# yuanqing-wang/stag

Hardware: AMD Instinct MI355X
Metric: aggregated edges/sec, stochastic-aggregation layer-forward, ogbn-arxiv-shaped CSR (higher is better)
Workload: dtype f32

## Files before the change

stag_amd/csrc/agg_kernel.hpp:

```cpp
#pragma once
#include "../../include/stag_hip.h"
#include "noise.hpp"

namespace stag {

struct AggArgs {
  const int32_t* indptr;
  const int32_t* indices;
  const int32_t* eid;
  const int32_t* nidx;
  int32_t n_rows;
  const float* x;
  int64_t ldx;
  int32_t D;
  uint32_t ldxb;
  uint32_t ldwb;
  uint32_t x_bytes;
  int32_t wide;
  const float* p0;
  const float* p1;
  float p0s, p1s;
  int32_t pmode;
  int32_t relu, in_norm;
  int32_t wgroup;
  PhiloxKey key;
  uint32_t pos_lo, pos_hi;
  uint32_t chunk_base;
  int32_t n_heavy;
  int32_t n_heavy_blocks;
  struct alignas(32) Walk {
    int32_t smask, sshift;
    int32_t jh_heavy;
    int32_t jh_light;
    int32_t sh;
    int32_t lbase;
    int32_t sl;
    int32_t n_total;
  } walk;
  const int32_t* xcd;
  const float* src_scale;
  const float* dst_scale;
  int32_t mean;
  float* out;
  float* outx[3];
  int32_t mc;
  uint64_t mc_stride;
  int64_t ldo;
  float* norm_scale_out;
  const float* xown;
  int64_t ldxo;
  const float* own_scale;
  float* eg0;
  float* eg1;
  float* dp_part;
  const stag_unit* units;
  const stag_unit* units_plan;
  int32_t n_units;
  const int32_t* long_rows;
  const int32_t* long_seg_ptr;
  int32_t n_long;
  int32_t n_seg;
  int32_t* seg_counters;
  float* ws;
  int32_t ws_stride;
  uint32_t ws_bytes;
};

__device__ __forceinline__ void load4(const float* p, int k0, int D, bool vec, float (&v)[4]) {
  if (vec) {
    const float4 t = *reinterpret_cast<const float4*>(p + k0);
    v[0] = t.x; v[1] = t.y; v[2] = t.z; v[3] = t.w;
  } else {
#pragma unroll
    for (int j = 0; j < 4; ++j) v[j] = (k0 + j < D) ? p[k0 + j] : 0.0f;
  }
}

__device__ __forceinline__ void store4(float* p, int k0, int D, bool vec, const float (&v)[4]) {
  if (vec) {
    *reinterpret_cast<float4*>(p + k0) = make_float4(v[0], v[1], v[2], v[3]);
  } else {
#pragma unroll
    for (int j = 0; j < 4; ++j)
      if (k0 + j < D) p[k0 + j] = v[j];
  }
}

__device__ __forceinline__ void store4_sc1(__amdgpu_buffer_rsrc_t rsrc, uint32_t off, int k0, int D,
                                           bool vec, const float (&v)[4]) {
  typedef unsigned int u32x4 __attribute__((ext_vector_type(4)));
  if (vec) {
    const u32x4 t = {__float_as_uint(v[0]), __float_as_uint(v[1]), __float_as_uint(v[2]),
                     __float_as_uint(v[3])};
    __builtin_amdgcn_raw_buffer_store_b128(t, rsrc, (int)off, 0, 16);
  } else {
#pragma unroll
    for (int j = 0; j < 4; ++j)
      if (k0 + j < D)
        __builtin_amdgcn_raw_buffer_store_b32(__float_as_uint(v[j]), rsrc, (int)(off + 4u * j), 0, 16);
  }
}

template <int NF, bool VEC>
__device__ __forceinline__ void kahan_sum_partials(const float* ws, int ws_stride, int s0, int s1,
                                                   int k0, int D, float (&sum)[4], float (&comp)[4]) {
  comp[0] = comp[1] = comp[2] = comp[3] = 0.f;
  sum[0] = sum[1] = sum[2] = sum[3] = 0.f;
#pragma unroll 1
  for (int s = s0; s < s1; s += NF) {
    float t[NF][4];
#pragma unroll
    for (int i = 0; i < NF; ++i) {
      if (s + i < s1) load4(ws + (int64_t)(s + i) * ws_stride, k0, D, VEC, t[i]);
      else t[i][0] = t[i][1] = t[i][2] = t[i][3] = 0.f;
    }
#pragma unroll
    for (int i = 0; i < NF; ++i)
#pragma unroll
      for (int q = 0; q < 4; ++q) {
        const float y = t[i][q] - comp[q];
        const float n = sum[q] + y;
        comp[q] = (n - sum[q]) - y;
        sum[q] = n;
      }
  }
}

__device__ __forceinline__ void agg_epilogue_extra(const AggArgs& a, float* out, int v, int deg, int k0,
                                                   bool vec, float (&acc)[4]);

constexpr int kCombineGroup = 16;
template <int NF, bool VEC, int LPE, int SLOTS>
__device__ __forceinline__ void two_level_sum(const float* ws, int ws_stride, int s0, int s1, int k0,
                                              int D, int sl, int slot0, float (&sum)[4]) {
  float comp[4] = {0.f, 0.f, 0.f, 0.f};
  sum[0] = sum[1] = sum[2] = sum[3] = 0.f;
#pragma unroll 1
  for (int g0 = s0; g0 < s1; g0 += kCombineGroup * SLOTS) {
    const int gs = g0 + sl * kCombineGroup;
    float gsum[4] = {0.f, 0.f, 0.f, 0.f}, gres[4] = {0.f, 0.f, 0.f, 0.f};
    if (gs < s1) {
      const int ge = min(gs + kCombineGroup, s1);
      kahan_sum_partials<NF, VEC>(ws, ws_stride, gs, ge, k0, D, gsum, gres);
    }
#pragma unroll
    for (int j = 0; j < SLOTS; ++j) {
      if (g0 + j * kCombineGroup < s1) {
#pragma unroll
// ... 377 lines not shown
      for (int o = 0; o < NX; ++o) fold_into(X.acc[o], X.comp[o], TX.acc[o]);
    }
    }
  }

  __device__ __forceinline__ void fold(const float (&t)[4]) { fold_into(acc, comp, t); }

  __device__ __forceinline__ void fold_into(float (&s)[4], float (&cmp)[4], const float (&t)[4]) const {
    if (kahan) {
#pragma unroll
      for (int q = 0; q < 4; ++q) {
        const float y = t[q] - cmp[q];
        const float sum = s[q] + y;
        cmp[q] = (sum - s[q]) - y;
        s[q] = sum;
      }
    } else {
#pragma unroll
      for (int q = 0; q < 4; ++q) s[q] += t[q];
    }
  }

  __device__ __forceinline__ void block_sums(EdgeRows<NB, PEDGE>& R, const EdgeIdx<NB>& I, int p0,
                                             float (&t)[MULT][4], float (&we)[NB][4]) {
#pragma unroll
    for (int m = 0; m < MULT; ++m) {
#pragma unroll
      for (int q = 0; q < 4; ++q) t[m][q] = 0.f;
#pragma unroll
      for (int j = m * BLK; j < (m + 1) * BLK; ++j) {
        if (p0 + j < pend) {
          edge_weight(R, I, j, we[j]);
          if (a.src_scale) {
            asm volatile("" ::: "memory");
#pragma unroll
            for (int q = 0; q < 4; ++q) R.xv[j][q] *= R.xs[j];
          }
#pragma unroll
          for (int q = 0; q < 4; ++q) t[m][q] = __builtin_fmaf(we[j][q], R.xv[j][q], t[m][q]);
        }
      }
    }
  }

  __device__ __forceinline__ void edge_weight(const EdgeRows<NB, PEDGE>& R, const EdgeIdx<NB>& I, int j,
                                              float (&w)[4]) {
    if constexpr (KIND == kNone) {
      w[0] = w[1] = w[2] = w[3] = 1.0f;
    } else if constexpr (KIND == kExplicit) {
      if (a.wgroup > 1) {
        const float* wr = a.p0 + (int64_t)I.ee[j] * (a.D / a.wgroup);
#pragma unroll
        for (int q = 0; q < 4; ++q) w[q] = (k0 + q < a.D) ? wr[(k0 + q) / a.wgroup] : 0.0f;
      } else {
        loadrow4(row_at(a.p0, I.ee[j], a.ldwb, koff, (a.wide & 2) != 0), k0, a.D, VEC, w);
      }
      if (a.relu & kFlagRelu) {
#pragma unroll
        for (int q = 0; q < 4; ++q) w[q] = fmaxf(w[q], 0.0f);
      }
    } else {
      if constexpr (PEDGE == 1) {
        const float s1 = (a.relu & kFlagLogScale) ? exp_scale(R.P.q1[j]) : R.P.q1[j];
#pragma unroll
        for (int q = 0; q < 4; ++q) { pa[q] = R.P.q0[j]; pb[q] = s1; }
        draw4<KIND>(I.nn[j], c1, key, pa, pb, a.relu, w);
        return;
      } else if constexpr (PEDGE == 2) {
        if (a.relu & kFlagLogScale) {
          float pbe[4];
#pragma unroll
          for (int q = 0; q < 4; ++q) pbe[q] = exp_scale(R.P.pb[j][q]);
          draw4<KIND>(I.nn[j], c1, key, R.P.pa[j], pbe, a.relu, w);
        } else {
          draw4<KIND>(I.nn[j], c1, key, R.P.pa[j], R.P.pb[j], a.relu, w);
        }
        return;
      }
      draw4<KIND>(I.nn[j], c1, key, pa, pb, a.relu, w);
    }
  }
};

template <int KIND, int LPE, bool VEC, int PEDGE, int SLOTS, int MULT, int NOUT = 1, bool MC = false, bool WN = false,
          bool NULLS = false>
__device__ __forceinline__ void agg_unit(const AggArgs& a, const int unit, const int c, const int sl,
                                         float (*dp_out)[4] = nullptr) {
  static_assert(LPE * SLOTS <= 64 && 64 % (LPE * SLOTS) == 0, "a unit's lanes stay inside one wave");
  static_assert(NOUT == 1 || SLOTS == 1, "the derivative outputs take the one-slot loop");
#ifndef STAG_BLK_EG
#define STAG_BLK_EG 1
#endif
#ifndef STAG_BLK_DP
#define STAG_BLK_DP 1
#endif
  constexpr int BLK = PEDGE == 3 ? STAG_BLK_EG : PEDGE == 4 ? STAG_BLK_DP : (KIND >= kNormal) ? STAG_BLK_RNG : STAG_BLK_MEM;
  constexpr int NB = BLK * MULT;

  const uint32_t chunk = blockIdx.y * LPE + c;
  const int k0 = (int)chunk * 4;
  if (k0 >= a.D) return;

  int v, b, len, slot = -1;
  if (a.units) {
    const int4 q = *reinterpret_cast<const int4*>(a.units + unit);
    v = q.x; b = q.y; len = q.z; slot = q.w;
    if constexpr (NULLS) {
      if (v < 0) return;
    }
  } else {
    v = unit;
    b = a.indptr[v];
    len = a.indptr[v + 1] - b;
  }

  if (len > STAG_PRIO_MIN_LEN) __builtin_amdgcn_s_setprio(2);
#ifdef STAG_TRACE
  uint64_t* trace = (!a.in_norm && a.norm_scale_out && blockIdx.y == 0 && c == 0 && sl == 0)
                        ? reinterpret_cast<uint64_t*>(a.norm_scale_out) + (int64_t)unit * 4 : nullptr;
  if (trace) { trace[0] = wall_clock64(); trace[1] = trace[2] = trace[3] = 0; }
#endif

  AggTeam<KIND, LPE, VEC, PEDGE, BLK, MULT, NOUT, MC, WN> T{
      a, (KIND >= kNormal) ? resolve_epoch(a.key) : a.key, k0, (uint32_t)k0 * 4u,
      (chunk + a.chunk_base) | (a.pos_hi << 20),
      b + len,
      __builtin_amdgcn_make_buffer_rsrc(const_cast<float*>(a.x), 0, (int)a.x_bytes, 0x00020000),
      (a.wide & 1) == 0 && a.x_bytes != 0,
      {a.p0s, a.p0s, a.p0s, a.p0s}, {a.p1s, a.p1s, a.p1s, a.p1s},
      {0.f, 0.f, 0.f, 0.f}, {0.f, 0.f, 0.f, 0.f}, {0.f, 0.f, 0.f, 0.f},
      len > kKahanMinLen};
  if constexpr (MC) {
#pragma unroll
    for (int o = 0; o < NOUT - 1; ++o) T.KX.k[o] = key_plus(T.key, (uint64_t)(o + 1) * a.mc_stride);
  }
  if constexpr (PEDGE == 3 || PEDGE == 4) {
    const int row = slot >= 0 ? a.long_rows[v] : v;
    const float os = a.own_scale ? a.own_scale[row] : 1.0f;
    if (PEDGE == 3 || a.xown) {
      load4(a.xown + (int64_t)row * a.ldxo, k0, a.D, VEC, T.XO.v);
    } else {
#pragma unroll
      for (int q = 0; q < 4; ++q) T.XO.v[q] = (k0 + q < a.D) ? 1.0f : 0.0f;
    }
#pragma unroll
    for (int q = 0; q < 4; ++q) T.XO.v[q] *= os;
  }
  if constexpr (KIND >= kNormal) {
    if (a.pmode == STAG_PARAM_PER_CHANNEL) {
      load4(a.p0, k0, a.D, VEC, T.pa);
      if (a.p1) load4(a.p1, k0, a.D, VEC, T.pb);
    }
  }

  const int pend = b + len;
  EdgeIdx<NB> I;
  EdgeRows<NB, PEDGE> R;
  {
    constexpr bool PREFETCH = STAG_IDX_PREFETCH && LPE <= ((KIND >= kNormal) ? STAG_PREFETCH_MAX_LPE : STAG_PREFETCH_MAX_LPE_MEM);
    if constexpr (SLOTS > 1) {
      constexpr int RB = SLOTS * NB;
      const int base = ((int)(threadIdx.x & 63) - sl * LPE) << 2;
      for (int r0 = b; r0 < pend; r0 += RB) {
        const int p0 = r0 + sl * NB;
#if STAG_LOAD_PRIO
        __builtin_amdgcn_s_setprio(3);
#endif
        T.fetch_idx(I, p0);
        T.pin_idx(I);
        T.fetch_rows(R, I, p0);
#if STAG_LOAD_PRIO
        if (len > STAG_PRIO_MIN_LEN) __builtin_amdgcn_s_setprio(2); else __builtin_amdgcn_s_setprio(0);
#endif
        float t[MULT][4], we[NB][4];
        T.block_sums(R, I, p0, t, we);
#pragma unroll
        for (int j = 0; j < SLOTS; ++j) {
#pragma unroll
          for (int m = 0; m < MULT; ++m) {
            const int pb = r0 + (j * MULT + m) * BLK;
            if (pb < pend) {
              float tj[4];
#pragma unroll
              for (int q = 0; q < 4; ++q)
                tj[q] = __int_as_float(__builtin_amdgcn_ds_bpermute(base + j * (LPE << 2), __float_as_int(t[m][q])));
              T.fold(tj);
              if (a.in_norm) {
#pragma unroll
                for (int e = 0; e < BLK; ++e) {
                  if (pb + e < pend) {
#pragma unroll
                    for (int q = 0; q < 4; ++q)
                      T.wsum[q] += __int_as_float(__builtin_amdgcn_ds_bpermute(
                          base + j * (LPE << 2), __float_as_int(we[m * BLK + e][q])));
                  }
                }
              }
            }
          }
        }
      }
    } else if constexpr (PREFETCH) {
    EdgeIdx<NB> In;
    T.fetch_idx(I, b);
    for (int p0 = b; p0 < pend; p0 += NB) {
#if STAG_LOAD_PRIO
      __builtin_amdgcn_s_setprio(3);
#endif
      T.pin_idx(I);
      T.fetch_rows(R, I, p0);
      if (p0 + NB < pend) T.fetch_idx(In, p0 + NB);
#if STAG_LOAD_PRIO
      if (len > STAG_PRIO_MIN_LEN) __builtin_amdgcn_s_setprio(2); else __builtin_amdgcn_s_setprio(0);
#endif
      T.compute(R, I, p0);
      I = In;
    }
    } else {
    for (int p0 = b; p0 < pend; p0 += NB) {
#if STAG_LOAD_PRIO
      __builtin_amdgcn_s_setprio(3);
#endif
      T.fetch_idx(I, p0);
      T.pin_idx(I);
      T.fetch_rows(R, I, p0);
#if STAG_LOAD_PRIO
      if (len > STAG_PRIO_MIN_LEN) __builtin_amdgcn_s_setprio(2); else __builtin_amdgcn_s_setprio(0);
#endif
      T.compute(R, I, p0);
    }
    }
  }

#ifdef STAG_TRACE
  if (trace) trace[1] = wall_clock64();
#endif
  if constexpr (PEDGE == 4) {
#pragma unroll
    for (int i = 0; i < 2; ++i)
#pragma unroll
      for (int q = 0; q < 4; ++q) dp_out[i][q] = T.DP.v[i][q];
// ... 153 lines not shown
    if constexpr (HS > 1) {
      if (blk < a.n_heavy_blocks) {
        const int unit = blk * TPBH + threadIdx.x / (LPE * HS);
        if (unit >= a.n_heavy) return;
        agg_unit<KIND, LPE, VEC, PEDGE, HS, STAG_HMULT>(a, unit, c, (threadIdx.x / LPE) % HS);
        return;
      }
      first = a.n_heavy;
      blk -= a.n_heavy_blocks;
    }
    const int unit = first + blk * TPB + threadIdx.x / LPE;
    if (unit >= a.n_units) return;
    agg_unit<KIND, LPE, VEC, PEDGE, 1, NOUT == 1 ? mult_of<KIND, LPE>() : 1, NOUT, MC, WN>(a, unit, c, 0);
  } else {
    const AggArgs::Walk w = a.walk;
    const int stripe = blockIdx.x & w.smask;
    int j = blockIdx.x >> w.sshift;
    int unit0, end;
    bool heavy = false;
    if (HS > 1 && j < w.jh_heavy) {
      heavy = true;
      unit0 = stripe * w.sh + j * TPBH;
      end = (stripe + 1) * w.sh;
    } else {
      if (HS > 1) j -= w.jh_heavy;
      if (j < w.jh_light) {
        unit0 = stripe * w.sh + j * TPB;
        end = (stripe + 1) * w.sh;
      } else {
        j -= w.jh_light;
        unit0 = w.lbase + stripe * w.sl + j * TPB;
        end = min(w.lbase + (stripe + 1) * w.sl, w.n_total);
      }
    }
    if constexpr (HS > 1) {
      if (heavy) {
        const int unit = unit0 + threadIdx.x / (LPE * HS);
        if (unit >= end) return;
        agg_unit<KIND, LPE, VEC, PEDGE, HS, STAG_HMULT, 1, false, false, true>(a, unit, c, (threadIdx.x / LPE) % HS);
        return;
      }
    }
    const int unit = unit0 + threadIdx.x / LPE;
    if (unit >= end) return;
#ifndef STAG_MULT_WALK_WIDE
#define STAG_MULT_WALK_WIDE 2
#endif
    constexpr int MULT_W = NOUT != 1 ? 1 : (KIND == kNone && PEDGE == 0 && LPE >= 64) ? STAG_MULT_WALK_WIDE : mult_of<KIND, LPE>();
    agg_unit<KIND, LPE, VEC, PEDGE, 1, MULT_W, NOUT, MC, WN, true>(a, unit, c, 0);
  }
}

template <int KIND, int LPE, bool VEC>
__global__ __launch_bounds__(STAG_BLOCK_THREADS, STAG_WAVES_PER_SIMD) void agg_dp_kernel(const AggArgs a) {
  constexpr int TEAMS = STAG_BLOCK_THREADS / LPE;
  __shared__ float s_dp[TEAMS][2][LPE * 4];
  const int c = threadIdx.x % LPE, tm = threadIdx.x / LPE;
  const int unit = blockIdx.x * TEAMS + tm;
  float dp[2][4] = {{0.f, 0.f, 0.f, 0.f}, {0.f, 0.f, 0.f, 0.f}};
  if (unit < a.n_units) agg_unit<KIND, LPE, VEC, 4, 1, 1>(a, unit, c, 0, dp);
#pragma unroll
  for (int i = 0; i < 2; ++i)
#pragma unroll
    for (int q = 0; q < 4; ++q) s_dp[tm][i][c * 4 + q] = dp[i][q];
  __syncthreads();
  float* part = a.dp_part + ((int64_t)blockIdx.y * gridDim.x + blockIdx.x) * (2 * LPE * 4);
  for (int i = threadIdx.x; i < 2 * LPE * 4; i += STAG_BLOCK_THREADS) {
    float sum = 0.f;
#pragma unroll
    for (int j = 0; j < TEAMS; ++j) sum += s_dp[j][i / (LPE * 4)][i % (LPE * 4)];
    part[i] = sum;
  }
}

template <int KIND>
hipError_t agg_launch(const AggArgs& a, bool vec, hipStream_t stream);

#ifndef STAG_XCD_PLANLESS
#define STAG_XCD_PLANLESS 1
#endif
#ifndef STAG_AGG_LDS_BYTES
#define STAG_AGG_LDS_BYTES 0
#endif
template <int KIND>
inline void agg_launch_small(const AggArgs& a_in, bool vec, int tiles, hipStream_t s) {
  AggArgs a = a_in;
  constexpr int LPE = 32, TPB = STAG_BLOCK_THREADS / LPE, TPBH = STAG_BLOCK_THREADS / (LPE * heavy_slots_of<KIND, LPE, true>());
  a.n_heavy_blocks = (a.n_heavy + TPBH - 1) / TPBH;
  const dim3 grid(a.n_heavy_blocks + (a.n_units - a.n_heavy + TPB - 1) / TPB, tiles), block(STAG_BLOCK_THREADS);
  if (grid.x == 0) return;
  if (vec) hipLaunchKernelGGL((agg_kernel<KIND, LPE, true, 0, 1, false, false, false, true>), grid, block, STAG_AGG_LDS_BYTES, s, a);
  else     hipLaunchKernelGGL((agg_kernel<KIND, LPE, false, 0, 1, false, false, false, true>), grid, block, STAG_AGG_LDS_BYTES, s, a);
}

template <int KIND, int LPE>
inline void agg_launch_shape(const AggArgs& a_in, bool vec, int pedge, int tiles, hipStream_t s) {
  if constexpr (LPE == 32 && heavy_slots_of<KIND, 32, true>() != heavy_slots_of<KIND, 32, false>()) {
    if (!a_in.outx[0] && !a_in.dp_part && pedge == 0 && !a_in.xcd && a_in.units && a_in.n_heavy > 0 &&
        a_in.n_units <= STAG_SMALL_UNITS) {
      agg_launch_small<KIND>(a_in, vec, tiles, s);
      return;
    }
  }
  AggArgs a = a_in;
  constexpr int TPB = STAG_BLOCK_THREADS / LPE;
  constexpr int HS = heavy_slots_of<KIND, LPE>();
  constexpr int TPBH = STAG_BLOCK_THREADS / (LPE * HS);
  const bool slotted = !(HS == 1 || a.outx[0] || pedge == 3 || a.dp_part);
  if (!slotted) a.n_heavy = 0;
  const bool plain = !a.outx[0] && !a.dp_part && pedge == 0;
  if (a.xcd && a.dp_part) { a.xcd = nullptr; a.units = a.units_plan; }
  a.n_heavy_blocks = (a.n_heavy + TPBH - 1) / TPBH;
  dim3 grid(a.n_heavy_blocks + (a.n_units - a.n_heavy + TPB - 1) / TPB, tiles);
  bool walk = false;
  AggArgs::Walk& w = a.walk;
  if (a.xcd) {
    walk = true;
    w.smask = STAG_XCD_STRIPES - 1; w.sshift = 3;
    w.jh_heavy = slotted ? (w.sh + TPBH - 1) / TPBH : 0;
    w.jh_light = slotted ? 0 : (w.sh + TPB - 1) / TPB;
    w.lbase = STAG_XCD_STRIPES * w.sh;
    w.n_total = STAG_XCD_STRIPES * (w.sh + w.sl);
    grid.x = STAG_XCD_STRIPES * (w.jh_heavy + w.jh_light + (w.sl + TPB - 1) / TPB);
  } else if (STAG_XCD_PLANLESS && !a.dp_part && !a.units && a.n_units >= STAG_XCD_STRIPES * TPB && a.n_units < (1 << 30)) {
    walk = true;
    w = AggArgs::Walk{STAG_XCD_STRIPES - 1, 3, 0, 0, 0, 0, 0, a.n_units};
    w.sl = ((a.n_units + STAG_XCD_STRIPES - 1) / STAG_XCD_STRIPES + TPB - 1) / TPB * TPB;
    grid.x = STAG_XCD_STRIPES * (w.sl / TPB);
  } else if (!plain && !a.dp_part) {
    walk = true;
    w = AggArgs::Walk{0, 0, 0, 0, a.n_heavy, a.n_heavy, a.n_units - a.n_heavy, a.n_units};
    w.jh_heavy = slotted ? a.n_heavy_blocks : 0;
    w.jh_light = slotted ? 0 : (w.sh + TPB - 1) / TPB;
    grid.x = w.jh_heavy + w.jh_light + (w.sl + TPB - 1) / TPB;
  }
  if (grid.x == 0) return;
  const dim3 block(STAG_BLOCK_THREADS);
  if constexpr (KIND >= kNormal) {
    if (a.mc && a.outx[2]) {
      if (vec) hipLaunchKernelGGL((agg_kernel<KIND, LPE, true, 0, 4, true, false, true>), grid, block, STAG_AGG_LDS_BYTES, s, a);
      else     hipLaunchKernelGGL((agg_kernel<KIND, LPE, false, 0, 4, true, false, true>), grid, block, STAG_AGG_LDS_BYTES, s, a);
      return;
    }
    if (a.mc && a.outx[0] && a.in_norm) {
      if (vec) hipLaunchKernelGGL((agg_kernel<KIND, LPE, true, 0, 2, true, true, true>), grid, block, STAG_AGG_LDS_BYTES, s, a);
      else     hipLaunchKernelGGL((agg_kernel<KIND, LPE, false, 0, 2, true, true, true>), grid, block, STAG_AGG_LDS_BYTES, s, a);
      return;
    }
    if (a.mc && a.outx[0]) {
      if (vec) hipLaunchKernelGGL((agg_kernel<KIND, LPE, true, 0, 2, true, false, true>), grid, block, STAG_AGG_LDS_BYTES, s, a);
      else     hipLaunchKernelGGL((agg_kernel<KIND, LPE, false, 0, 2, true, false, true>), grid, block, STAG_AGG_LDS_BYTES, s, a);
      return;
    }
  }
  if constexpr (KIND == kNormal || KIND == kUniform) {
    if (a.outx[0]) {
      if (vec) hipLaunchKernelGGL((agg_kernel<KIND, LPE, true, 0, 3, false, false, true>), grid, block, STAG_AGG_LDS_BYTES, s, a);
      else     hipLaunchKernelGGL((agg_kernel<KIND, LPE, false, 0, 3, false, false, true>), grid, block, STAG_AGG_LDS_BYTES, s, a);
      return;
    }
  }
  if constexpr (KIND == kNormal || KIND == kUniform) {
    if (a.dp_part) {
      if (vec) hipLaunchKernelGGL((agg_dp_kernel<KIND, LPE, true>), grid, block, STAG_AGG_LDS_BYTES, s, a);
      else     hipLaunchKernelGGL((agg_dp_kernel<KIND, LPE, false>), grid, block, STAG_AGG_LDS_BYTES, s, a);
      return;
    }
    if (pedge == 3) {
      if (vec) hipLaunchKernelGGL((agg_kernel<KIND, LPE, true, 3, 1, false, false, true>), grid, block, STAG_AGG_LDS_BYTES, s, a);
      else     hipLaunchKernelGGL((agg_kernel<KIND, LPE, false, 3, 1, false, false, true>), grid, block, STAG_AGG_LDS_BYTES, s, a);
      return;
    }
  }
  if constexpr (KIND >= kNormal) {
    if (pedge == 1) {
      if (vec) hipLaunchKernelGGL((agg_kernel<KIND, LPE, true, 1, 1, false, false, true>), grid, block, STAG_AGG_LDS_BYTES, s, a);
      else     hipLaunchKernelGGL((agg_kernel<KIND, LPE, false, 1, 1, false, false, true>), grid, block, STAG_AGG_LDS_BYTES, s, a);
      return;
    }
    if (pedge == 2) {
      if (vec) hipLaunchKernelGGL((agg_kernel<KIND, LPE, true, 2, 1, false, false, true>), grid, block, STAG_AGG_LDS_BYTES, s, a);
      else     hipLaunchKernelGGL((agg_kernel<KIND, LPE, false, 2, 1, false, false, true>), grid, block, STAG_AGG_LDS_BYTES, s, a);
      return;
    }
  }
  if (walk) {
    if (vec) hipLaunchKernelGGL((agg_kernel<KIND, LPE, true, 0, 1, false, false, true>), grid, block, STAG_AGG_LDS_BYTES, s, a);
    else     hipLaunchKernelGGL((agg_kernel<KIND, LPE, false, 0, 1, false, false, true>), grid, block, STAG_AGG_LDS_BYTES, s, a);
    return;
  }
  if (vec) hipLaunchKernelGGL((agg_kernel<KIND, LPE, true, 0>), grid, block, STAG_AGG_LDS_BYTES, s, a);
  else     hipLaunchKernelGGL((agg_kernel<KIND, LPE, false, 0>), grid, block, STAG_AGG_LDS_BYTES, s, a);
}

template <int KIND>
inline hipError_t agg_launch_impl(const AggArgs& a, bool vec, hipStream_t s) {
  const int nchunk = (a.D + 3) / 4;
  const int pedge = (KIND < kNormal) ? 0 : a.pmode == STAG_PARAM_PER_EDGE1 ? (a.eg0 ? 3 : 1)
                    : a.pmode == STAG_PARAM_PER_EDGE ? 2 : 0;
  int lpe = 1;
  while (lpe < nchunk && lpe < 64) lpe <<= 1;
  const int tiles = (nchunk + lpe - 1) / lpe;
  switch (lpe) {
    case 64: agg_launch_shape<KIND, 64>(a, vec, pedge, tiles, s); break;
    case 32: agg_launch_shape<KIND, 32>(a, vec, pedge, tiles, s); break;
    case 16: agg_launch_shape<KIND, 16>(a, vec, pedge, tiles, s); break;
    case 8:  agg_launch_shape<KIND, 8>(a, vec, pedge, tiles, s); break;
    case 4:  agg_launch_shape<KIND, 4>(a, vec, pedge, tiles, s); break;
    case 2:  agg_launch_shape<KIND, 2>(a, vec, pedge, tiles, s); break;
    default: agg_launch_shape<KIND, 1>(a, vec, pedge, tiles, s); break;
  }
  return hipGetLastError();
}

}
```

stag_amd/csrc/api.hip:

```cpp
#include <algorithm>
#include <cmath>
#include <cstring>
#include <vector>

#include "../../include/stag_hip.h"
#include "agg_kernel.hpp"
#include "agg_max.hpp"

using namespace stag;

namespace stag {
template <int KIND>
hipError_t agg_launch(const AggArgs& a, bool vec, hipStream_t stream);
}

namespace {

inline bool aligned16(const void* p) { return (reinterpret_cast<uintptr_t>(p) & 15u) == 0; }

int check_spec(const stag_noise_spec* s, int64_t n_edges = 1, int32_t Dn = 0) {
  if (!s) return STAG_EINVAL;
  if (s->kind < STAG_NOISE_NONE || s->kind > STAG_NOISE_BERNOULLI) return STAG_EINVAL;
  if (s->kind == STAG_NOISE_EXPLICIT && !s->p0 && n_edges > 0) return STAG_EINVAL;
  if (s->deriv < 0 || s->deriv > 2 || s->chunk_base < 0 || s->chunk_base >= (1 << 20)) return STAG_EINVAL;
// ... 657 lines not shown
      block_ptr_host[j * STAG_XCD_STRIPES + x + 1] = at;
    }
  return STAG_OK;
}
}
}

int stag_plan_blocks_xcd(const stag_unit* units_host, int32_t n_units, int64_t n_edges, int32_t fine, int32_t max_edges,
                         int32_t max_units, stag_unit* units_out_host, int32_t* block_ptr_host, int32_t* n_blocks_out) {
  if (n_units < 0 || n_edges < 0 || fine < 1 || fine > STAG_XCD_FINE_MAX || max_edges <= 0 || max_units <= 0 ||
      !n_blocks_out || (n_units > 0 && !units_host) || ((units_out_host == nullptr) != (block_ptr_host == nullptr)))
    return STAG_EINVAL;
  return plan_blocks_xcd_impl(units_host, n_units, fine, XcdKeyByPosition{n_edges > 0 ? n_edges : 1, STAG_XCD_STRIPES * fine},
                              max_edges, max_units, units_out_host, block_ptr_host, n_blocks_out);
}

int stag_plan_blocks_xcd_ranges(const stag_unit* units_host, int32_t n_units, const int64_t* cuts_host,
                                const int32_t* keys_host, int32_t n_ranges, int32_t fine, int32_t max_edges, int32_t max_units,
                                stag_unit* units_out_host, int32_t* block_ptr_host, int32_t* n_blocks_out) {
  if (n_units < 0 || fine < 1 || fine > STAG_XCD_FINE_MAX || max_edges <= 0 || max_units <= 0 || !n_blocks_out ||
      (n_units > 0 && !units_host) || ((units_out_host == nullptr) != (block_ptr_host == nullptr)) ||
      !xcd_ranges_ok(cuts_host, keys_host, n_ranges, fine)) return STAG_EINVAL;
  return plan_blocks_xcd_impl(units_host, n_units, fine, XcdKeyByRange{cuts_host, keys_host, n_ranges}, max_edges, max_units,
                              units_out_host, block_ptr_host, n_blocks_out);
}

size_t stag_plan_workspace_bytes(int32_t n_seg, int32_t D, int32_t in_norm) {
  if (n_seg <= 0 || D <= 0) return 0;
  return (size_t)n_seg * (size_t)D * (in_norm ? 2u : 1u) * sizeof(float);
}

int stag_philox_raw(uint64_t seed, uint64_t offset, int64_t pos0, int64_t n_pos, int32_t n_chunk,
                    uint32_t* out, void* stream) {
  if (!out || n_pos < 0 || n_chunk <= 0 || !aligned16(out)) return STAG_EINVAL;
  const int64_t n = n_pos * n_chunk;
  if (n == 0) return STAG_OK;
  stag_noise_spec s{};
  s.seed = seed; s.offset = offset;
  hipLaunchKernelGGL(philox_raw_kernel, dim3((unsigned)((n + 255) / 256)), dim3(256), 0,
                     (hipStream_t)stream, make_key(&s), pos0, n_pos, n_chunk, out);
  return hipGetLastError() == hipSuccess ? STAG_OK : STAG_EIO;
}

int stag_normal_tables(float* rad, float* cosv, float* sinv, void* stream) {
  if (!rad || !cosv || !sinv) return STAG_EINVAL;
  hipLaunchKernelGGL(normal_tables_kernel, dim3((1u << 23) / 256), dim3(256), 0, (hipStream_t)stream, rad, cosv, sinv);
  return hipGetLastError() == hipSuccess ? STAG_OK : STAG_EIO;
}

struct EdgeGradOut {
  const float* xown;
  int64_t ldxo;
  float* eg0;
  float* eg1;
  float* dp_part;
};
static int agg_common(const stag_csr* csr, const stag_plan* plan, const float* x, int64_t ldx,
                      int32_t D, const stag_noise_spec* spec, int32_t reduce, const float* src_scale,
                      const float* dst_scale, float* out, int64_t ldo, float* norm_scale_out,
                      int nout, float* const* extra, int mc, uint64_t mc_stride, void* stream,
                      const EdgeGradOut* eg = nullptr) {
  int rc = check_csr(csr);
  if (rc) return rc;
  rc = check_spec(spec, csr->n_edges, D);
  if (rc) return rc;
  if (D <= 0 || (ldx != 0 && ldx < D) || ldo < D) return STAG_EINVAL;
  if (reduce != STAG_REDUCE_SUM && reduce != STAG_REDUCE_MEAN) return STAG_EINVAL;
  if (csr->n_dst == 0) return STAG_OK;
  if (!out && !norm_scale_out && !eg) return STAG_EINVAL;
  if (csr->n_edges > 0 && !x) return STAG_EINVAL;

  AggArgs a{};
  a.indptr = csr->indptr; a.indices = csr->indices; a.eid = csr->eid; a.nidx = csr->nidx;
  a.n_rows = csr->n_dst;
  a.x = x; a.ldx = ldx; a.D = D;
  a.ldxb = (uint32_t)(ldx * 4); a.ldwb = (uint32_t)D * 4u;
  {
    const uint64_t xbytes = (uint64_t)csr->n_src * (uint64_t)ldx * 4u;
    const uint64_t wbytes = (uint64_t)csr->n_edges * (uint64_t)D * 4u;
    const bool x_narrow = xbytes < (1ull << 32) && csr->n_src < (1 << 24) && (uint64_t)ldx * 4u < (1u << 24);
    const bool w_narrow = wbytes < (1ull << 32) && csr->n_edges < (1 << 24) && (uint64_t)D * 4u < (1u << 24);
    a.wide = (x_narrow ? 0 : 1) | (w_narrow ? 0 : 2);
    a.x_bytes = x_narrow ? (uint32_t)(ldx == 0 ? (uint64_t)D * 4u : xbytes) : 0u;
  }
  const bool logs = spec->kind == STAG_NOISE_NORMAL && spec->p1_log;
  a.p0 = spec->p0; a.p1 = spec->p1; a.p0s = spec->p0_scalar; a.p1s = logs ? expf(spec->p1_scalar) : spec->p1_scalar;
  a.pmode = spec->kind >= STAG_NOISE_NORMAL ? spec->param_mode : 0;
  a.relu = (spec->relu ? kFlagRelu : 0) | (spec->deriv << kDerivShift) | (logs ? kFlagLogScale : 0);
  a.in_norm = spec->in_norm;
  a.wgroup = (spec->kind == STAG_NOISE_EXPLICIT && spec->group > 1) ? spec->group : 1;
  if (a.wgroup > 1 && (D % a.wgroup != 0 || spec->in_norm)) return STAG_EINVAL;
  a.key = make_key(spec);
  a.pos_lo = (uint32_t)((uint64_t)spec->pos_base & 0xFFFFFFFFull);
  a.pos_hi = (uint32_t)((uint64_t)spec->pos_base >> 32);
  a.chunk_base = (uint32_t)spec->chunk_base;
  if (spec->kind >= STAG_NOISE_NORMAL && (uint64_t)a.pos_lo + (uint64_t)csr->n_edges > (1ull << 32))
    return STAG_ENOSYS;
  a.src_scale = src_scale; a.dst_scale = dst_scale; a.mean = (reduce == STAG_REDUCE_MEAN);
  a.out = out; a.ldo = ldo; a.norm_scale_out = norm_scale_out;
  for (int o = 0; o + 1 < nout; ++o) a.outx[o] = extra[o];
  a.mc = mc; a.mc_stride = mc_stride;
  if (eg) {
    a.xown = eg->xown; a.ldxo = eg->ldxo; a.own_scale = dst_scale; a.eg0 = eg->eg0; a.eg1 = eg->eg1;
    a.dp_part = eg->dp_part;
  }

  const bool use_plan = plan && plan->n_units > 0;
  const bool has_segs = use_plan && plan->n_seg > 0;
  a.n_units = csr->n_dst;
  if (use_plan) {
    if (!plan->units || !aligned16(plan->units)) return STAG_EINVAL;
    a.units = a.units_plan = static_cast<const stag_unit*>(plan->units);
    a.n_units = plan->n_units;
    if (plan->n_heavy < 0 || plan->n_heavy > plan->n_units) return STAG_EINVAL;
    a.n_heavy = plan->n_heavy;
    if (plan->xcd_order && !(eg && eg->dp_part)) {
      const int64_t sh = plan->xcd_stride_heavy, sl = plan->xcd_stride_light;
      if (!aligned16(plan->xcd_order) || sh < 0 || sl < 0 || sh > plan->n_heavy || sl > plan->n_units ||
          STAG_XCD_STRIPES * (sh + sl) < plan->n_units || STAG_XCD_STRIPES * (sh + sl) > 0x7FFFFFFFll) return STAG_EINVAL;
      a.xcd = plan->xcd_order;
      a.units = reinterpret_cast<const stag_unit*>(plan->xcd_order + STAG_XCD_HEADER);
      a.walk.sh = (int32_t)sh;
      a.walk.sl = (int32_t)sl;
    }
  }
  if (has_segs) {
    if (!plan->long_rows || !plan->long_seg_ptr || !plan->workspace || !plan->seg_counters)
      return STAG_EINVAL;
    const size_t need = stag_plan_workspace_bytes(plan->n_seg, nout * D, spec->in_norm);
    if (plan->workspace_bytes < need) return STAG_ENOMEM;
    a.long_rows = plan->long_rows; a.long_seg_ptr = plan->long_seg_ptr;
    if (need >= (1ull << 32)) return STAG_ENOSYS;
    a.ws = plan->workspace; a.ws_stride = D * nout * (spec->in_norm ? 2 : 1); a.ws_bytes = (uint32_t)need;
    a.n_long = plan->n_long; a.seg_counters = plan->seg_counters; a.n_seg = plan->n_seg;
  }

  bool vec = (D % 4 == 0) && (ldx % 4 == 0) && (ldo % 4 == 0) && aligned16(x) && (!out || aligned16(out));
  if (norm_scale_out) vec = vec && aligned16(norm_scale_out);
  for (int o = 0; o + 1 < nout; ++o) vec = vec && aligned16(extra[o]);
  if (spec->kind == STAG_NOISE_EXPLICIT) vec = vec && aligned16(spec->p0);
  if (spec->kind >= STAG_NOISE_NORMAL && spec->param_mode != STAG_PARAM_SCALAR &&
      spec->param_mode != STAG_PARAM_PER_EDGE1)
    vec = vec && aligned16(spec->p0) && (!spec->p1 || aligned16(spec->p1));
  if (has_segs) vec = vec && aligned16(plan->workspace);
  if (eg && eg->xown) vec = vec && aligned16(eg->xown) && (eg->ldxo % 4 == 0);

  hipStream_t s = (hipStream_t)stream;
  auto launch = [&](const AggArgs& args) -> hipError_t {
    switch (spec->kind) {
      case STAG_NOISE_NONE: return agg_launch<kNone>(args, vec, s);
      case STAG_NOISE_EXPLICIT: return agg_launch<kExplicit>(args, vec, s);
      case STAG_NOISE_NORMAL: return agg_launch<kNormal>(args, vec, s);
      case STAG_NOISE_UNIFORM: return agg_launch<kUniform>(args, vec, s);
      default: return agg_launch<kBernoulli>(args, vec, s);
    }
  };
  if (launch(a) != hipSuccess) return STAG_EIO;
  return STAG_OK;
}

int stag_agg_fwd(const stag_csr* csr, const stag_plan* plan, const float* x, int64_t ldx,
                 int32_t D, const stag_noise_spec* spec, int32_t reduce, const float* src_scale,
                 const float* dst_scale, float* out, int64_t ldo, float* norm_scale_out,
                 void* stream) {
  return agg_common(csr, plan, x, ldx, D, spec, reduce, src_scale, dst_scale, out, ldo, norm_scale_out,
                    1, nullptr, 0, 0, stream);
// ... 426 lines not shown
```

Before: 11.53 billion.

## Add specialized plain forward kernel for scalar-param sampled noise aggregation

Adds a dedicated kernel path for the common forward case: scalar noise parameters, no per-edge params, no extra outputs, vector loads. The path walks edges two at a time, loads indices through a buffer resource, draws noise with packed two-wide float math, and accumulates in packed fp32 registers. The kernel is pinned to a fixed waves-per-EU target to control register pressure and occupancy. It adds more template instantiations and compiled files, and can be turned off with an environment variable.

```diff
diff --git a/stag_amd/csrc/agg_kernel.hpp b/stag_amd/csrc/agg_kernel.hpp
--- a/stag_amd/csrc/agg_kernel.hpp
+++ b/stag_amd/csrc/agg_kernel.hpp
@@ -1,6 +1,7 @@
 #pragma once
 #include "../../include/stag_hip.h"
 #include "noise.hpp"
+#include <stdlib.h>
 
 namespace stag {
 
@@ -64,6 +65,7 @@
   float* ws;
   int32_t ws_stride;
   uint32_t ws_bytes;
+  uint32_t idx_bytes;
 };
 
 __device__ __forceinline__ void load4(const float* p, int k0, int D, bool vec, float (&v)[4]) {
@@ -607,8 +609,11 @@
   }
 };
 
+template <int KIND, int LPE, bool RELU, class TEAM>
+__device__ __forceinline__ void plain_walk(const AggArgs& a, TEAM& T, int b, int pend, int len);
+
 template <int KIND, int LPE, bool VEC, int PEDGE, int SLOTS, int MULT, int NOUT = 1, bool MC = false, bool WN = false,
-          bool NULLS = false>
+          bool NULLS = false, int PLAIN = 0>
 __device__ __forceinline__ void agg_unit(const AggArgs& a, const int unit, const int c, const int sl,
                                          float (*dp_out)[4] = nullptr) {
   static_assert(LPE * SLOTS <= 64 && 64 % (LPE * SLOTS) == 0, "a unit's lanes stay inside one wave");
@@ -681,7 +686,10 @@
   const int pend = b + len;
   EdgeIdx<NB> I;
   EdgeRows<NB, PEDGE> R;
-  {
+  if constexpr (PLAIN != 0) {
+    static_assert(SLOTS == 1 && MULT == 1 && NOUT == 1 && PEDGE == 0 && VEC && BLK == 2, "the plain forward launch");
+    plain_walk<KIND, LPE, (PLAIN & 2) != 0>(a, T, b, pend, len);
+  } else {
     constexpr bool PREFETCH = STAG_IDX_PREFETCH && LPE <= ((KIND >= kNormal) ? STAG_PREFETCH_MAX_LPE : STAG_PREFETCH_MAX_LPE_MEM);
     if constexpr (SLOTS > 1) {
       constexpr int RB = SLOTS * NB;
@@ -1001,6 +1009,23 @@
 #ifndef STAG_AGG_LDS_BYTES
 #define STAG_AGG_LDS_BYTES 0
 #endif
+inline bool plain_launch_ok(const AggArgs& a, bool vec, int pedge) {
+  return vec && pedge == 0 && a.pmode == STAG_PARAM_SCALAR && !a.outx[0] && !a.dp_part && !a.mc && a.out &&
+         !a.src_scale && !a.in_norm && !a.nidx && (a.relu & ~(kFlagRelu | kFlagLogScale)) == 0 &&
+         (a.wide & 1) == 0 && a.x_bytes != 0 && a.idx_bytes != 0;
+}
+
+template <int KIND>
+void agg_launch_plain(const AggArgs& a, int lpe, bool walk, dim3 grid, hipStream_t s);
+
+inline bool plain_enabled() {
+#if defined(STAG_TRACE) || defined(STAG_EXP_NO_ROWS)
+  return false;
+#endif
+  const char* e = getenv("STAG_AGG_PLAIN");
+  return !(e && e[0] == '0' && e[1] == 0);
+}
+
 template <int KIND>
 inline void agg_launch_small(const AggArgs& a_in, bool vec, int tiles, hipStream_t s) {
   AggArgs a = a_in;
@@ -1103,6 +1128,12 @@
       return;
     }
   }
+  if constexpr (KIND >= kNormal && (LPE == 32 || LPE == 64)) {
+    if (plain_launch_ok(a, vec, pedge) && plain_enabled()) {
+      agg_launch_plain<KIND>(a, LPE, walk, grid, s);
+      return;
+    }
+  }
   if (walk) {
     if (vec) hipLaunchKernelGGL((agg_kernel<KIND, LPE, true, 0, 1, false, false, true>), grid, block, STAG_AGG_LDS_BYTES, s, a);
     else     hipLaunchKernelGGL((agg_kernel<KIND, LPE, false, 0, 1, false, false, true>), grid, block, STAG_AGG_LDS_BYTES, s, a);
diff --git a/stag_amd/csrc/agg_plain.hpp b/stag_amd/csrc/agg_plain.hpp
--- /dev/null
+++ b/stag_amd/csrc/agg_plain.hpp
@@ -0,0 +1,150 @@
+#pragma once
+#include "agg_kernel.hpp"
+
+namespace stag {
+
+#ifndef STAG_PLAIN_WAVES
+#define STAG_PLAIN_WAVES 7
+#endif
+
+typedef float f32x2_t __attribute__((ext_vector_type(2)));
+
+template <int KIND, bool RELU>
+__device__ __forceinline__ void plain_draw4(uint32_t c0, uint32_t c1, const PhiloxKey& key, f32x2_t p0, float p1,
+                                            f32x2_t (&w)[2]) {
+  uint32_t r[4];
+  philox4x32_10(c0, c1, key, r);
+  const f32x2_t s = {p1, p1};
+  if constexpr (KIND == kNormal) {
+    const f32x2_t z01 = f32x2_t{bm_cos(r[1]), bm_sin(r[1])} * bm_radius(r[0]);
+    const f32x2_t z23 = f32x2_t{bm_cos(r[3]), bm_sin(r[3])} * bm_radius(r[2]);
+    w[0] = __builtin_elementwise_fma(s, z01, p0);
+    w[1] = __builtin_elementwise_fma(s, z23, p0);
+  } else if constexpr (KIND == kUniform) {
+    w[0] = __builtin_elementwise_fma(s, f32x2_t{u01(r[0]), u01(r[1])}, p0);
+    w[1] = __builtin_elementwise_fma(s, f32x2_t{u01(r[2]), u01(r[3])}, p0);
+  } else {
+    w[0] = f32x2_t{u01(r[0]) < p0.x ? 1.0f : 0.0f, u01(r[1]) < p0.y ? 1.0f : 0.0f};
+    w[1] = f32x2_t{u01(r[2]) < p0.x ? 1.0f : 0.0f, u01(r[3]) < p0.y ? 1.0f : 0.0f};
+  }
+  if constexpr (RELU) {
+    w[0] = __builtin_elementwise_max(w[0], f32x2_t{0.f, 0.f});
+    w[1] = __builtin_elementwise_max(w[1], f32x2_t{0.f, 0.f});
+  }
+}
+
+template <int KIND, int LPE, bool RELU, class TEAM>
+__device__ __forceinline__ void plain_walk(const AggArgs& a, TEAM& T, const int b, const int pend, const int len) {
+  const __amdgpu_buffer_rsrc_t ri =
+      __builtin_amdgcn_make_buffer_rsrc(const_cast<int32_t*>(a.indices), 0, (int)a.idx_bytes, 0x00020000);
+  f32x2_t p0 = {a.p0s, a.p0s};
+  asm volatile("" : "+v"(p0));
+  const float p1 = KIND == kUniform ? a.p1s - a.p0s : a.p1s;
+  const uint32_t pos1 = a.pos_lo + 1u;
+  f32x2_t s01 = {0.f, 0.f}, s23 = {0.f, 0.f}, c01 = {0.f, 0.f}, c23 = {0.f, 0.f};
+  const int pend1 = pend - 1;
+  for (int p = b; p < pend; p += 2) {
+    const bool two = p < pend1;
+#if STAG_LOAD_PRIO
+    __builtin_amdgcn_s_setprio(3);
+#endif
+    const int u0 = (int)__builtin_amdgcn_raw_buffer_load_b32(ri, p << 2, 0, 0);
+    int u1;
+    if (two) u1 = (int)__builtin_amdgcn_raw_buffer_load_b32(ri, (p << 2) + 4, 0, 0);
+    uint32_t n0 = a.pos_lo + (uint32_t)p, n1 = pos1 + (uint32_t)p;
+    asm volatile("" : "+v"(n0));
+    asm volatile("" : "+v"(n1));
+    u32x4_t x1;
+    const u32x4_t x0 = __builtin_amdgcn_raw_buffer_load_b128(T.rx, (int)(__umul24((uint32_t)u0, a.ldxb) + T.koff), 0, STAG_X_AUX);
+    if (two) x1 = __builtin_amdgcn_raw_buffer_load_b128(T.rx, (int)(__umul24((uint32_t)u1, a.ldxb) + T.koff), 0, STAG_X_AUX);
+#if STAG_LOAD_PRIO
+    if (len > STAG_PRIO_MIN_LEN) __builtin_amdgcn_s_setprio(2); else __builtin_amdgcn_s_setprio(0);
+#endif
+    f32x2_t w0[2], w1[2];
+    plain_draw4<KIND, RELU>(n0, T.c1, T.key, p0, p1, w0);
+    if (two) plain_draw4<KIND, RELU>(n1, T.c1, T.key, p0, p1, w1);
+    const f32x2_t zero = {0.f, 0.f};
+    f32x2_t t01 = __builtin_elementwise_fma(w0[0], f32x2_t{__uint_as_float(x0.x), __uint_as_float(x0.y)}, zero);
+    f32x2_t t23 = __builtin_elementwise_fma(w0[1], f32x2_t{__uint_as_float(x0.z), __uint_as_float(x0.w)}, zero);
+    if (two) {
+      asm volatile("" ::: "memory");
+      t01 = __builtin_elementwise_fma(w1[0], f32x2_t{__uint_as_float(x1.x), __uint_as_float(x1.y)}, t01);
+      t23 = __builtin_elementwise_fma(w1[1], f32x2_t{__uint_as_float(x1.z), __uint_as_float(x1.w)}, t23);
+    }
+    if (T.kahan) {
+      const f32x2_t y01 = t01 - c01, y23 = t23 - c23;
+      const f32x2_t n01 = s01 + y01, n23 = s23 + y23;
+      c01 = (n01 - s01) - y01; c23 = (n23 - s23) - y23;
+      s01 = n01; s23 = n23;
+    } else {
+      s01 += t01; s23 += t23;
+    }
+  }
+  T.acc[0] = s01.x; T.acc[1] = s01.y; T.acc[2] = s23.x; T.acc[3] = s23.y;
+}
+
+template <int KIND, int LPE, bool RELU, bool WALK>
+__global__ __launch_bounds__(STAG_BLOCK_THREADS)
+__attribute__((amdgpu_waves_per_eu(STAG_PLAIN_WAVES, STAG_PLAIN_WAVES))) void agg_plain_kernel(const AggArgs a_in) {
+  static_assert(KIND >= kNormal && (LPE == 32 || LPE == 64), "the plain launch: sampled noise, 32 or 64 lanes per row");
+  static_assert(heavy_slots_of<KIND, LPE>() == 1 && mult_of<KIND, LPE>() == 1, "wide shapes walk one slot, one block");
+  AggArgs a = a_in;
+  if constexpr (WALK) {
+    STAG_PIN_S(a.walk.smask); STAG_PIN_S(a.walk.sshift); STAG_PIN_S(a.walk.jh_light);
+    STAG_PIN_S(a.walk.sh); STAG_PIN_S(a.walk.lbase); STAG_PIN_S(a.walk.sl); STAG_PIN_S(a.walk.n_total);
+  }
+  STAG_PIN_S(a.D); STAG_PIN_S(a.units); STAG_PIN_S(a.indptr); STAG_PIN_S(a.indices);
+  STAG_PIN_S(a.x); STAG_PIN_S(a.ldxb); STAG_PIN_S(a.x_bytes); STAG_PIN_S(a.idx_bytes);
+  STAG_PIN_S(a.p0s); STAG_PIN_S(a.p1s);
+  STAG_PIN_S(a.key.k0); STAG_PIN_S(a.key.k1); STAG_PIN_S(a.key.o0); STAG_PIN_S(a.key.o1); STAG_PIN_S(a.key.epoch);
+  STAG_PIN_S(a.pos_lo); STAG_PIN_S(a.pos_hi); STAG_PIN_S(a.chunk_base);
+  a.relu = RELU ? kFlagRelu : 0;
+  a.in_norm = 0; a.norm_scale_out = nullptr;
+  a.src_scale = nullptr;
+  a.nidx = nullptr; a.eid = nullptr;
+  a.pmode = STAG_PARAM_SCALAR; a.p0 = nullptr; a.p1 = nullptr;
+  a.wide = 0;
+  __builtin_assume(a.x_bytes != 0);
+  __builtin_assume(a.out != nullptr);
+
+  const int c = threadIdx.x % LPE;
+  constexpr int TPB = STAG_BLOCK_THREADS / LPE;
+  if constexpr (!WALK) {
+    const int unit = blockIdx.x * TPB + threadIdx.x / LPE;
+    if (unit >= a.n_units) return;
+    agg_unit<KIND, LPE, true, 0, 1, 1, 1, false, false, false, RELU ? 3 : 1>(a, unit, c, 0);
+  } else {
+    const AggArgs::Walk w = a.walk;
+    const int stripe = blockIdx.x & w.smask;
+    int j = blockIdx.x >> w.sshift;
+    int unit0, end;
+    if (j < w.jh_light) {
+      unit0 = stripe * w.sh + j * TPB;
+      end = (stripe + 1) * w.sh;
+    } else {
+      j -= w.jh_light;
+      unit0 = w.lbase + stripe * w.sl + j * TPB;
+      end = min(w.lbase + (stripe + 1) * w.sl, w.n_total);
+    }
+    const int unit = unit0 + threadIdx.x / LPE;
+    if (unit >= end) return;
+    agg_unit<KIND, LPE, true, 0, 1, 1, 1, false, false, true, RELU ? 3 : 1>(a, unit, c, 0);
+  }
+}
+
+template <int KIND>
+inline void agg_launch_plain_impl(const AggArgs& a, int lpe, bool walk, dim3 grid, hipStream_t s) {
+  const dim3 block(STAG_BLOCK_THREADS);
+  const bool relu = (a.relu & kFlagRelu) != 0;
+#define STAG_PLAIN_GO(L, R, W) hipLaunchKernelGGL((agg_plain_kernel<KIND, L, R, W>), grid, block, STAG_AGG_LDS_BYTES, s, a)
+  if (lpe == 32) {
+    if (walk) { if (relu) STAG_PLAIN_GO(32, true, true); else STAG_PLAIN_GO(32, false, true); }
+    else      { if (relu) STAG_PLAIN_GO(32, true, false); else STAG_PLAIN_GO(32, false, false); }
+  } else {
+    if (walk) { if (relu) STAG_PLAIN_GO(64, true, true); else STAG_PLAIN_GO(64, false, true); }
+    else      { if (relu) STAG_PLAIN_GO(64, true, false); else STAG_PLAIN_GO(64, false, false); }
+  }
+#undef STAG_PLAIN_GO
+}
+
+}
diff --git a/stag_amd/csrc/agg_plain_bernoulli.hip b/stag_amd/csrc/agg_plain_bernoulli.hip
--- /dev/null
+++ b/stag_amd/csrc/agg_plain_bernoulli.hip
@@ -0,0 +1,8 @@
+#include "agg_plain.hpp"
+
+namespace stag {
+template <>
+void agg_launch_plain<kBernoulli>(const AggArgs& a, int lpe, bool walk, dim3 grid, hipStream_t stream) {
+  agg_launch_plain_impl<kBernoulli>(a, lpe, walk, grid, stream);
+}
+}
diff --git a/stag_amd/csrc/agg_plain_normal.hip b/stag_amd/csrc/agg_plain_normal.hip
--- /dev/null
+++ b/stag_amd/csrc/agg_plain_normal.hip
@@ -0,0 +1,8 @@
+#include "agg_plain.hpp"
+
+namespace stag {
+template <>
+void agg_launch_plain<kNormal>(const AggArgs& a, int lpe, bool walk, dim3 grid, hipStream_t stream) {
+  agg_launch_plain_impl<kNormal>(a, lpe, walk, grid, stream);
+}
+}
diff --git a/stag_amd/csrc/agg_plain_uniform.hip b/stag_amd/csrc/agg_plain_uniform.hip
--- /dev/null
+++ b/stag_amd/csrc/agg_plain_uniform.hip
@@ -0,0 +1,8 @@
+#include "agg_plain.hpp"
+
+namespace stag {
+template <>
+void agg_launch_plain<kUniform>(const AggArgs& a, int lpe, bool walk, dim3 grid, hipStream_t stream) {
+  agg_launch_plain_impl<kUniform>(a, lpe, walk, grid, stream);
+}
+}
diff --git a/stag_amd/csrc/api.hip b/stag_amd/csrc/api.hip
--- a/stag_amd/csrc/api.hip
+++ b/stag_amd/csrc/api.hip
@@ -763,6 +763,7 @@
     const bool w_narrow = wbytes < (1ull << 32) && csr->n_edges < (1 << 24) && (uint64_t)D * 4u < (1u << 24);
     a.wide = (x_narrow ? 0 : 1) | (w_narrow ? 0 : 2);
     a.x_bytes = x_narrow ? (uint32_t)(ldx == 0 ? (uint64_t)D * 4u : xbytes) : 0u;
+    a.idx_bytes = csr->n_edges < (1 << 30) ? (uint32_t)csr->n_edges * 4u : 0u;
   }
   const bool logs = spec->kind == STAG_NOISE_NORMAL && spec->p1_log;
   a.p0 = spec->p0; a.p1 = spec->p1; a.p0s = spec->p0_scalar; a.p1s = logs ? expf(spec->p1_scalar) : spec->p1_scalar;
```

After: 12.14 billion, median of 6. +5.3%, better.
